# ZHENGXi-git/TC-VIML

Measured on NVIDIA B200. Metric: linearized_factors_per_s, higher is better.
Workload: dtype f64

## Files before the change

### tc-viml_b200/csrc/assemble2.cuh

```cuda
#pragma once

namespace stream {

constexpr int PMAX = 12;
constexpr int FMAXP = 4096;
constexpr int PT = 64;
constexpr int PT_MAX = 512;
constexpr int TASK_T = 180;
constexpr int TASK_F = 24;
constexpr int LTASK = 32;
constexpr int AW = 4;
constexpr int LACC_W = 14;
constexpr int STAGE_D = 1024;
constexpr int LACC_D = TASK_F * LACC_W;
constexpr int WORK_D = STAGE_D + LACC_D + 192;

struct PlanPtrs {
  int4* hdr;
  int4* tasks;
  uint32_t* slots;
  uint32_t* finfo;
  uint32_t* lslots;
  int* any_irregular;
};

__host__ __device__ inline int task_base(int a0_rel, int w, int F) { return a0_rel / 64 + w * (F / TASK_F + PMAX + 4); }

__device__ __forceinline__ int warp_incl_scan(int v, int lane) {
#pragma unroll
  for (int d = 1; d < 32; d <<= 1) {
    const int t = __shfl_up_sync(0xffffffffu, v, d);
    if (lane >= d) v += t;
  }
  return v;
}

__global__ void __launch_bounds__(PT_MAX) plan_kernel(LinearizeArgs A, PlanPtrs PL) {
  extern __shared__ __align__(16) unsigned char plan_raw[];
  __shared__ int gcount[PMAX + 2], grun[PMAX + 2], lcount[PMAX + 1], lrun[PMAX + 1];
  __shared__ int s_bad, s_big, s_ntasks, s_nlslots;
  const int tid = threadIdx.x, lane = tid & 31, warp = tid >> 5, w = blockIdx.x;
  const int P = A.P, F = A.F, NTH = (int)blockDim.x;
  uint32_t* fmask = reinterpret_cast<uint32_t*>(plan_raw);
  uint32_t* fanchor = fmask + F;
  uint32_t* cexcl = fanchor + F;
  uint16_t* ford = reinterpret_cast<uint16_t*>(cexcl + F + 1);
  uint16_t* fid = ford + ((F + 1) & ~1);
  const int a0 = A.pf_window_offset[w], nf = A.pf_window_offset[w + 1] - a0;
  const int b0 = A.NL > 0 ? A.lf_window_offset[w] : 0, nl = A.NL > 0 ? A.lf_window_offset[w + 1] - b0 : 0;
  const int a0r = a0 - (int)A.pf_begin, b0r = b0 - (int)A.lf_begin;
  for (int f = tid; f < F; f += NTH) fmask[f] = 0u, fanchor[f] = 0xffu;
  for (int e = tid; e < F * P; e += NTH) fid[e] = 0xffff;
  if (tid < PMAX + 2) gcount[tid] = 0;
  if (tid < PMAX + 1) lcount[tid] = 0;
  if (tid == 0) s_bad = s_big = (nf > 65534 || nl > 65534 || nf < 0 || nl < 0) ? 1 : 0, s_ntasks = 0, s_nlslots = 0;
  __syncthreads();
  const int nfs = s_big ? 0 : nf;
  for (int k = tid; k < nfs; k += NTH) {
    const uint32_t ix = A.pf_idx[a0 + k];
    const int i = ix & 0xff, j = (ix >> 8) & 0xff, l = ix >> 16;
    if (i >= P || j >= P || l >= F || i == j) {
      s_bad = 1;
      continue;
    }
    const uint32_t old = atomicOr(&fmask[l], 1u << j);
    const uint32_t an = atomicCAS(&fanchor[l], 0xffu, (uint32_t)i);
    if (((old >> j) & 1u) || (an != 0xffu && an != (uint32_t)i)) s_bad = 1;
    fid[l * P + j] = (uint16_t)k;
  }
  __syncthreads();
  if (s_bad) {
    if (tid == 0) {
      PL.hdr[w] = make_int4(0, 0, 1, 0);
      atomicOr(PL.any_irregular, 1);
    }
    return;
  }
  uint32_t* lsl = PL.lslots + 2 * (size_t)b0r;
  if (warp == 0) {
    for (int f0 = 0; f0 < F; f0 += 32) {
      const int f = f0 + lane;
      const int key = f < F ? (fanchor[f] == 0xffu ? P : (int)fanchor[f]) : 64 + lane;
      const unsigned m = __match_any_sync(0xffffffffu, key);
      if (f < F && (m & ((1u << lane) - 1u)) == 0u) gcount[key] += __popc(m);
      __syncwarp();
    }
    {
      const int c = lane <= P ? gcount[lane] : 0;
      const int inc = warp_incl_scan(c, lane);
      if (lane <= P) grun[lane] = inc - c;
    }
    __syncwarp();
    for (int f0 = 0; f0 < F; f0 += 32) {
      const int f = f0 + lane;
      const int key = f < F ? (fanchor[f] == 0xffu ? P : (int)fanchor[f]) : 64 + lane;
      const unsigned m = __match_any_sync(0xffffffffu, key);
      const int rank = __popc(m & ((1u << lane) - 1u));
      if (f < F) ford[grun[key] + rank] = (uint16_t)f;
      __syncwarp();
      if (f < F && rank == 0) grun[key] += __popc(m);
      __syncwarp();
    }
    int carry = 0;
    for (int p0 = 0; p0 < F; p0 += 32) {
      const int p = p0 + lane;
      const int c = p < F ? __popc(fmask[ford[p]]) : 0;
      const int inc = warp_incl_scan(c, lane);
      if (p < F) cexcl[p] = (uint32_t)(carry + inc - c);
      carry += __shfl_sync(0xffffffffu, inc, 31);
    }
    if (lane == 0) cexcl[F] = (uint32_t)carry;
    __syncwarp();
    const int tb = task_base(a0r, w, F);
    int pos = 0, t = 0;
    bool at_group_start = true;
    while (pos < F) {
      const int p = pos + lane;
      const int c = p < F ? (int)(cexcl[p + 1] - cexcl[p]) : 0x10000;
      const int inc = warp_incl_scan(c, lane);
      const unsigned okm = __ballot_sync(0xffffffffu, inc <= TASK_T && p < F && lane < TASK_F);
      int n = okm == 0xffffffffu ? 32 : __ffs(~okm) - 1;
      n = max(n, 1);
      n = min(n, F - pos);
      const int an = p < F ? (fanchor[ford[p]] == 0xffu ? P : (int)fanchor[ford[p]]) : -1;
      const unsigned same = __ballot_sync(0xffffffffu, an == __shfl_sync(0xffffffffu, an, 0));
      const int na = same == 0xffffffffu ? 33 : __ffs(~same) - 1;
      int excl = 0;
      if (na <= n) {
        n = na;
        excl = at_group_start ? 1 : 0;
        at_group_start = true;
      } else {
        at_group_start = false;
      }
      if (lane == 0) PL.tasks[tb + t] = make_int4(2 * (int)cexcl[pos], 0, pos, n | (excl << 16));
      pos += n, ++t;
    }
    if (lane == 0) s_ntasks = t;
  } else if (warp == 1 && nl > 0) {
    bool bad = false;
    for (int k0 = 0; k0 < nl; k0 += 32) {
      const int k = k0 + lane;
      int key = k < nl ? A.lf_frame[b0 + k] : 64 + lane;
      if (k < nl && (key < 0 || key >= P)) bad = true, key = 96 + lane;
      const unsigned m = __match_any_sync(0xffffffffu, key);
      if (k < nl && key < P && (m & ((1u << lane) - 1u)) == 0u) lcount[key] += __popc(m);
      __syncwarp();
    }
    if (__any_sync(0xffffffffu, bad)) {
      if (lane == 0) s_bad = 1;
    } else {
      const int c = lane < P ? ((lcount[lane] + 1) & ~1) : 0;
      const int inc = warp_incl_scan(c, lane);
      if (lane < P) {
        lrun[lane] = inc - c;
        if (lcount[lane] & 1) lsl[inc - 1] = 0xffffu | ((uint32_t)lane << 16);
      }
      if (lane == 31) s_nlslots = inc;
      __syncwarp();
      for (int k0 = 0; k0 < nl; k0 += 32) {
        const int k = k0 + lane;
        const int key = k < nl ? A.lf_frame[b0 + k] : 64 + lane;
        const unsigned m = __match_any_sync(0xffffffffu, key);
        const int rank = __popc(m & ((1u << lane) - 1u));
        if (k < nl) lsl[lrun[key] + rank] = (uint32_t)k | ((uint32_t)key << 16);
        __syncwarp();
        if (k < nl && rank == 0) lrun[key] += __popc(m);
        __syncwarp();
      }
    }
  }
  __syncthreads();
  if (s_bad) {
    if (tid == 0) {
      PL.hdr[w] = make_int4(0, 0, 1, 0);
      atomicOr(PL.any_irregular, 1);
    }
    return;
  }
  const int tb = task_base(a0r, w, F), nt = s_ntasks;
  uint32_t* sl_w = PL.slots + 2 * (size_t)a0r;
  for (int t = warp; t < nt; t += NTH / 32) {
    int4 tk = PL.tasks[tb + t];
    const int p = tk.z + lane;
    const bool on = lane < (tk.w & 0xffff);
    const int l = on ? ford[p] : 0;
    const uint32_t m = on ? fmask[l] : 0u;
    const int an = (on && m) ? (int)fanchor[l] : 0xff;
    if (on) PL.finfo[(size_t)w * F + p] = (uint32_t)l | (m << 16) | ((uint32_t)(an & 15) << 28);
    uint32_t* sl = sl_w + tk.x;
    int off = 0;
    const unsigned lt = (1u << lane) - 1u;
    unsigned im = __reduce_or_sync(0xffffffffu, an < P ? 1u << an : 0u);
    while (im) {
      const int i = __ffs(im) - 1;
      im &= im - 1;
      unsigned jm = __reduce_or_sync(0xffffffffu, an == i ? m : 0u);
      while (jm) {
        const int j = __ffs(jm) - 1;
        jm &= jm - 1;
        const bool mine = an == i && ((m >> j) & 1u);
        const unsigned b = __ballot_sync(0xffffffffu, mine);
        const int n = __popc(b);
        const uint32_t key = ((uint32_t)i << 21) | ((uint32_t)j << 25);
        if (mine) sl[off + __popc(b & lt)] = (uint32_t)fid[l * P + j] | ((uint32_t)lane << 16) | key;
        if ((n & 1) && lane == 0) sl[off + n] = 0xffffu | key;
        off += (n + 1) & ~1;
      }
    }
    if (lane == 0) PL.tasks[tb + t].y = off;
  }
  if (tid == 0) PL.hdr[w] = make_int4(nt, s_nlslots, 0, 0);
}

enum Kind { K_LL = 0, K_HH, K_LH, K_LE, K_HE, K_EE, K_BL, K_BH, K_BE, K_NKIND };

struct Tables {
  uint32_t seg[128];
  uint32_t lo[64];
  uint32_t ee[32];
  uint32_t line[32];
};

constexpr uint32_t tab_entry(int R, int C, int kind, int off, bool neg) {
  const int tile = (R < 8 && C < 8) ? 0 : (R < 8 ? 1 : 2);
  return 0x80000000u | (uint32_t)(tile * 64 + (R & 7) * 8 + (C & 7)) | ((uint32_t)kind << 8) | ((uint32_t)off << 12) |
         (neg ? (1u << 18) : 0u);
}

constexpr int col_type(int c) { return c < 3 ? 0 : (c < 6 ? 1 : (c < 9 ? 2 : (c < 15 ? 3 : 4))); }
// ... 80 lines not shown

__device__ __forceinline__ int swz(int f) { return ((f & 1) << 2) ^ ((f >> 1) & 3); }

struct Dest {
  int src;
  int off;
  int kind;
  unsigned sign;
};
__device__ __forceinline__ Dest decode(uint32_t e) {
  Dest d;
  d.src = (e >> 31) ? (int)(e & 0xff) : -1;
  d.off = (e >> 12) & 63;
  d.kind = (e >> 8) & 15;
  d.sign = ((e >> 18) & 1u) << 31;
  return d;
}
template <int ROUNDS>
__device__ __forceinline__ void scatter(const double* __restrict__ patch, const Dest* tab, double* __restrict__ Hc,
                                        int mybase, bool store_lh = false) {
  double v[ROUNDS];
  double* dst[ROUNDS];
#pragma unroll
  for (int r = 0; r < ROUNDS; ++r) {
    const int base = __shfl_sync(0xffffffffu, mybase, tab[r].kind);
    dst[r] = Hc + base + tab[r].off;
    const double x = patch[tab[r].src >= 0 ? tab[r].src : 0];
    v[r] = __hiloint2double(__double2hiint(x) ^ (int)tab[r].sign, __double2loint(x));
  }
#pragma unroll
  for (int r = 0; r < ROUNDS; ++r) {
    if (tab[r].src >= 0) {
      if (store_lh && tab[r].kind == K_LH) *dst[r] = v[r];
      else atomicAdd(dst[r], v[r]);
    }
  }
}

__device__ __forceinline__ int kind_base(int rs, int cs, bool isb, int lo, int hi, int NB, int boff) {
  const int e = NB - 1;
  const int x = rs == 0 ? lo : (rs == 1 ? hi : e), y = cs == 0 ? lo : (cs == 1 ? hi : e);
  return isb ? boff + 6 * x : blk(x, y, NB) * 36;
}

__device__ __forceinline__ void put_patch(double* __restrict__ patch, int lane, const double (&G)[6]) {
  double2* p2 = reinterpret_cast<double2*>(patch);
  const int o = (lane >> 2) * 4 + (lane & 3);
  p2[o] = make_double2(G[0], G[1]);
  p2[32 + o] = make_double2(G[2], G[3]);
  p2[64 + o] = make_double2(G[4], G[5]);
}

template <bool MODE_A>
__global__ void __maxnreg__(168) assemble_kernel(LinearizeArgs A, PlanPtrs PL, int use_tma) {
  extern __shared__ __align__(16) unsigned char asm_raw[];
  __shared__ int s_next;
  constexpr int NT = AW * 32;
  const int tid = threadIdx.x, lane = tid & 31, warp = tid >> 5, w = blockIdx.x;
  const int P = A.P, F = A.F, D = A.D, NB = P + 1;
  const int nblk = NB * (NB + 1) / 2, boff = nblk * 36;
  const int hc_n = (boff + D + 1) & ~1;
  const int cstride = P * kPoseCache + kExCache;
  double* __restrict__ Hc = reinterpret_cast<double*>(asm_raw);
  double* __restrict__ cache = Hc + hc_n;
  double* __restrict__ work0 = cache + cstride;
  double* __restrict__ stage = work0 + warp * WORK_D;
  double* __restrict__ lacc = stage + STAGE_D;
  double* __restrict__ patch = lacc + LACC_D;

  const int4 hdr = PL.hdr[w];
  const int a0 = A.pf_window_offset[w];
  const int b0 = A.NL > 0 ? A.lf_window_offset[w] : 0;
  double* __restrict__ Hpp = A.out.H_pp + (size_t)w * D * D;
  double* __restrict__ Hlp = A.out.H_lp + (size_t)w * F * D;
  double* __restrict__ Hll = A.out.H_ll + (size_t)w * F;
  double* __restrict__ bp = A.out.b_p + (size_t)w * D;
  double* __restrict__ bl = A.out.b_l + (size_t)w * F;
  const double2* __restrict__ gc = reinterpret_cast<const double2*>(A.cache + (size_t)w * cstride);
  double2 cpre[3];
#pragma unroll
  for (int q = 0; q < 3; ++q) cpre[q] = tid + q * NT < cstride / 2 ? gc[tid + q * NT] : make_double2(0.0, 0.0);
  uint32_t traw[7];
#pragma unroll
  for (int r = 0; r < 3; ++r) traw[r] = g_tables.seg[32 * r + lane];
#pragma unroll
  for (int r = 0; r < 2; ++r) traw[3 + r] = g_tables.lo[32 * r + lane];
  traw[5] = g_tables.ee[lane], traw[6] = g_tables.line[lane];
  if (hdr.z) {
    for (int e = tid; e < D * D; e += NT) Hpp[e] = 0.0;
    for (int e = tid; e < F * D; e += NT) Hlp[e] = 0.0;
    for (int e = tid; e < F; e += NT) Hll[e] = 0.0, bl[e] = 0.0;
    for (int e = tid; e < D; e += NT) bp[e] = 0.0;
    return;
  }
  {
    double2* z = reinterpret_cast<double2*>(Hc);
    for (int e = tid; e < hc_n / 2; e += NT) z[e] = make_double2(0.0, 0.0);
    double2* c2 = reinterpret_cast<double2*>(cache);
#pragma unroll
    for (int q = 0; q < 3; ++q)
      if (tid + q * NT < cstride / 2) c2[tid + q * NT] = cpre[q];
    for (int e = tid + 3 * NT; e < cstride / 2; e += NT) c2[e] = gc[e];
  }
  if (tid == 0) s_next = 0;
  Dest tab_seg[3], tab_lo[2], tab_ee[1], tab_line[1];
#pragma unroll
  for (int r = 0; r < 3; ++r) tab_seg[r] = decode(traw[r]);
#pragma unroll
  for (int r = 0; r < 2; ++r) tab_lo[r] = decode(traw[3 + r]);
  tab_ee[0] = decode(traw[5]);
  tab_line[0] = decode(traw[6]);
  const int kb_rs = lane < K_NKIND ? (0x24904 >> (2 * lane)) & 3 : 0, kb_cs = lane < K_NKIND ? (0xA94 >> (2 * lane)) & 3 : 0;
  const bool kb_isb = lane >= K_BL && lane < K_NKIND;
  __syncthreads();

  const int ntask = hdr.x, nlsl = hdr.y, nltask = (nlsl + LTASK - 1) / LTASK;
  const int tb = task_base(a0 - (int)A.pf_begin, w, F);
  const uint32_t* __restrict__ sl_w = PL.slots + 2 * (size_t)(a0 - (int)A.pf_begin);
  const uint32_t* __restrict__ lsl_w = PL.lslots + 2 * (size_t)(b0 - (int)A.lf_begin);
  const int g = lane >> 2, kk = lane & 3;
  const int gx = g ^ ((kk >> 1) << 2);
  const double* __restrict__ frag0 = stage + (kk >> 1) * 32 + (kk & 1);
  const unsigned full = 0xffffffffu;
  const int upr = 3 * NB;
  const int ru1 = 32 + (lane & 7), rb0 = (lane * 11) >> 5, rb1 = (ru1 * 43) >> 7;
  const int rp0 = lane - 3 * rb0, rp1 = ru1 - 3 * rb1;

  double E[2] = {0.0, 0.0};
  for (;;) {
    int t = 0;
    if (lane == 0) t = atomicAdd(&s_next, 1);
    t = __shfl_sync(full, t, 0);
    if (t >= ntask + nltask) break;
    if (t < ntask) {
      const int4 tk = PL.tasks[tb + t];
      const int n_slots = tk.y, n_feats = tk.w & 0xffff;
      const bool excl = (tk.w >> 16) != 0;
      const uint32_t fi = lane < n_feats ? PL.finfo[(size_t)w * F + tk.z + lane] : 0u;
      {
        double2* z = reinterpret_cast<double2*>(lacc);
        for (int q = lane; q < LACC_D / 2; q += 32) z[q] = make_double2(0.0, 0.0);
      }
      __syncwarp();
      const uint32_t* __restrict__ sl = sl_w + tk.x;
      double G[6] = {0, 0, 0, 0, 0, 0}, R[4] = {0, 0, 0, 0};
// ... 229 lines not shown
      const int br = r / 6, bc = c / 6, rr = r - 6 * br, cc = c - 6 * bc;
      const int lo = min(br, bc), hi = max(br, bc);
      const bool tr = br > bc || (br == bc && rr > cc);
      int a = tr ? cc : rr, b = tr ? rr : cc;
      if (lo != hi && hi < NB - 1 && a < 3 && b < a) { const int t = a; a = b, b = t; }
      Hpp[e] = Hc[blk(lo, hi, NB) * 36 + a * 6 + b];
    }
  } else {
    double2* __restrict__ Hf2 = reinterpret_cast<double2*>(Hf);
    const int Dh = D / 2;
    int br = 0, row0 = 0, rown = NB;
    for (int e = tid; e < nblk * 18; e += NT) {
      const int q = (e * 3641) >> 16, k = e - 18 * q;
      const int rr = (k * 11) >> 5, cp = k - 3 * rr, cc = 2 * cp;
      while (q >= row0 + rown) row0 += rown, --rown, ++br;
      const int bc = br + (q - row0);
      const double* __restrict__ sb = Hc + q * 36;
      if (br != bc) {
        const bool pp = bc < NB - 1;
        auto at = [&](int a, int b) { return sb[(pp && a < 3 && b < a) ? b * 6 + a : a * 6 + b]; };
        Hf2[(6 * br + rr) * Dh + 3 * bc + cp] = make_double2(at(rr, cc), at(rr, cc + 1));
        Hf2[(6 * bc + rr) * Dh + 3 * br + cp] = make_double2(at(cc, rr), at(cc + 1, rr));
      } else {
        Hf2[(6 * br + rr) * Dh + 3 * bc + cp] =
            make_double2(rr <= cc ? sb[rr * 6 + cc] : sb[cc * 6 + rr], rr <= cc + 1 ? sb[rr * 6 + cc + 1] : sb[(cc + 1) * 6 + rr]);
      }
    }
  }
  if (staged) {
    for (int e = tid; e < D; e += NT) Hf[D * D + e] = Hc[boff + e];
  } else {
    for (int e = tid; e < D; e += NT) bp[e] = Hc[boff + e];
  }
  if (use_tma) {
    asm volatile("fence.proxy.async.shared::cta;" ::: "memory");
    __syncthreads();
    if (tid == 0) {
      const uint32_t s0 = (uint32_t)__cvta_generic_to_shared(Hf);
      asm volatile("cp.async.bulk.global.shared::cta.bulk_group [%0], [%1], %2;" ::"l"(Hpp), "r"(s0), "r"((uint32_t)(D * D * 8))
                   : "memory");
      asm volatile("cp.async.bulk.global.shared::cta.bulk_group [%0], [%1], %2;" ::"l"(bp), "r"(s0 + (uint32_t)(D * D * 8)),
                   "r"((uint32_t)(D * 8))
                   : "memory");
      asm volatile("cp.async.bulk.commit_group;" ::: "memory");
      asm volatile("cp.async.bulk.wait_group.read 0;" ::: "memory");
    }
  } else if (staged) {
    __syncthreads();
    for (int e = tid; e < D * D; e += NT) Hpp[e] = Hf[e];
    for (int e = tid; e < D; e += NT) bp[e] = Hf[D * D + e];
  }
}

template <bool MODE_A>
__global__ void __launch_bounds__(128) irregular_kernel(LinearizeArgs A, PlanPtrs PL) {
  if (!*PL.any_irregular) return;
  const int cstride = A.P * kPoseCache + kExCache;
  for (int w = blockIdx.x; w < A.W; w += gridDim.x) {
    if (!PL.hdr[w].z) continue;
    const double* cw = A.cache + (size_t)w * cstride;
    const int a0 = A.pf_window_offset[w], a1 = A.pf_window_offset[w + 1];
    for (int64_t k = a0 + threadIdx.x; k < a1; k += blockDim.x) {
      const uint32_t pk = A.pf_idx[k];
      const int i = pk & 0xff, j = (pk >> 8) & 0xff, f = pk >> 16;
      if (i >= A.P || j >= A.P || f >= A.F) continue;
      const double4 ob = reinterpret_cast<const double4*>(A.pf_obs)[k];
      const double piz = A.pf_pts_i_z ? A.pf_pts_i_z[k] : 1.0;
      PointJac J;
      eval_point(A, cw, i, j, A.inv_depth[(size_t)w * A.F + f], ob.x, ob.y, piz, ob.z, ob.w, J);
      if (MODE_A) {
        if (A.out.pf_residual) reinterpret_cast<double2*>(A.out.pf_residual)[k] = make_double2(J.r[0], J.r[1]);
        if (A.out.pf_jac_pose_i) store_jac7(A.out.pf_jac_pose_i + 14 * k, J.a);
        if (A.out.pf_jac_pose_j) store_jac7(A.out.pf_jac_pose_j + 14 * k, J.b);
        if (A.out.pf_jac_ex) store_jac7(A.out.pf_jac_ex + 14 * k, J.c);
        if (A.out.pf_jac_feat) reinterpret_cast<double2*>(A.out.pf_jac_feat)[k] = make_double2(J.d[0], J.d[1]);
      }
      point_atomics(A, w, i, j, f, J, true, false);
    }
    if (A.NL > 0) {
      const int b0 = A.lf_window_offset[w], b1 = A.lf_window_offset[w + 1];
      for (int64_t k = b0 + threadIdx.x; k < b1; k += blockDim.x) {
        const int frame = A.lf_frame[k];
        if (frame < 0 || frame >= A.P) continue;
        double g9[9];
#pragma unroll
        for (int c = 0; c < 9; ++c) g9[c] = A.lf_geom[(size_t)c * A.NL_stride + k];
        LineJac J;
        eval_line(A, cw, frame, g9, J);
        if (MODE_A) {
          if (A.out.lf_residual) reinterpret_cast<double2*>(A.out.lf_residual)[k] = make_double2(J.r[0], J.r[1]);
          if (A.out.lf_jac_pose) store_jac7(A.out.lf_jac_pose + 14 * k, J.a);
        }
        line_atomics(A, w, frame, J);
      }
    }
  }
}

}
```

### tc-viml_b200/csrc/common.cuh

```cuda
#pragma once
#include <cuda_runtime.h>

#include <cstdint>
#include <cstdio>
#include <string>
#include <utility>
#include <vector>

#include "viml.h"

#define VIML_TRY_CUDA(ctx, expr)                                                              \
  do {                                                                                        \
    cudaError_t e__ = (expr);                                                                 \
    if (e__ != cudaSuccess) {                                                                 \
      (ctx)->err = std::string(#expr) + ": " + cudaGetErrorString(e__);                      \
      return VIML_ERR_CUDA;                                                                   \
    }                                                                                         \
  } while (0)

struct DeviceArena {
  char* base = nullptr;
  size_t cap = 0, used = 0;
  cudaError_t reserve(size_t bytes) {
    used = 0;
// ... 10 lines not shown
  T* take(size_t count) {
    const size_t bytes = (count * sizeof(T) + 255) & ~size_t(255);
    T* p = (T*)(base + used);
    used += bytes;
    return p;
  }
  static size_t padded(size_t bytes) { return (bytes + 255) & ~size_t(255); }
  void release() {
    if (base) cudaFree(base);
    base = nullptr;
    cap = used = 0;
  }
};

struct viml_ctx {
  int device = 0;
  int sm_count = 148;
  cudaStream_t stream = nullptr;
  cudaStream_t copy_stream = nullptr;
  cudaStream_t copy_stream2 = nullptr;
  cudaEvent_t ev_a = nullptr, ev_b = nullptr;
  cudaStream_t aux_stream = nullptr;
  cudaEvent_t ev_fork = nullptr, ev_join = nullptr;
  viml_config cfg{};
  std::string err;
  int64_t launches = 0;
  double cos_th = 0.0;
  int nan_angle_passes = 0;
  double* d_map = nullptr;
  int64_t n_map = 0;
  bool map_set = false;
  double* d_map_sorted = nullptr;
  int32_t* d_map_orig = nullptr;
  double* d_tile_sphere = nullptr;
  double* d_group_sphere = nullptr;
  int64_t n_tiles = 0;
  uint32_t* d_fov_slots = nullptr;
  int32_t* d_fov_slot_count = nullptr;
  int64_t fov_words = 0;
  unsigned long long* d_assoc_stats = nullptr;
  DeviceArena in_arena, out_arena, scratch, scratch2, scratch3, gn_in, gn_out, s_full;
  bool schur_splitk = false;
  char *h_stage_in = nullptr, *h_stage_out = nullptr;
  size_t h_stage_in_cap = 0, h_stage_out_cap = 0;
  void* nccl_lib = nullptr;
  bool brute_cull = false;
  bool force_generic = false;
  bool prof = false;
  std::vector<std::pair<cudaEvent_t, cudaEvent_t>> prof_events[VIML_NUM_KERNELS];
};

enum KernelId {
  K_PREP = 0, K_POINTS, K_LINES, K_ASSEMBLE, K_SCHUR, K_CAMPOSE, K_CULL, K_SCAN, K_FILL, K_PROJECT, K_MATCH,
  K_MARG, K_MICRO, K_PLAN, K_IRREGULAR, K_GN, K_COUNT
};
static_assert(K_COUNT <= VIML_NUM_KERNELS, "raise VIML_NUM_KERNELS");

struct LaunchScope {
  viml_ctx* ctx;
  cudaEvent_t stop = nullptr;
  cudaStream_t on;
  LaunchScope(viml_ctx* c, int id, cudaStream_t st = nullptr) : ctx(c), on(st ? st : c->stream) {
    ctx->launches++;
    if (ctx->prof) {
      cudaEvent_t a, b;
      cudaEventCreate(&a);
      cudaEventCreate(&b);
      cudaEventRecord(a, on);
      ctx->prof_events[id].emplace_back(a, b);
      stop = b;
    }
  }
  ~LaunchScope() {
    if (stop) cudaEventRecord(stop, on);
  }
};

constexpr int kMapTile = 64;
constexpr int kPoseCache = 42;
constexpr int kExCache = 24;
constexpr int PC_P = 0, PC_R = 3, PC_RINV = 12, PC_M = 21, PC_RL = 30, PC_TL = 39;
constexpr int EC_TIC = 0, EC_RIC = 3, EC_RICINV = 12, EC_RTT = 21;

struct LinearizeArgs {
  int W, P, F, D;
  int64_t NP, NL;
  int64_t pf_begin, lf_begin;
  int64_t NL_stride;
  const double* poses;
  const double* ex_pose;
  const double* inv_depth;
  const int32_t* pf_window_offset;
  const uint32_t* pf_idx;
  const double* pf_obs;
  const double* pf_pts_i_z;
  const int32_t* lf_window_offset;
  const int32_t* lf_frame;
  const double* lf_geom;
  double* cache;
  viml_linearize_out out;
  double sqrt_info, cauchy_a, inv_cauchy_a2, fx, fy, cx, cy;
  uint32_t flags;
};

struct DenseArgs {
  int X;
  int64_t ND;
// ... 102 lines not shown
```

### tc-viml_b200/csrc/linearize_kernels.cu

```cuda
#include <cstdlib>
#include <vector>

#include "common.cuh"

namespace {

__device__ __forceinline__ void quat_to_rot(double w, double x, double y, double z, double* R) {
  const double tx = 2.0 * x, ty = 2.0 * y, tz = 2.0 * z;
  const double twx = tx * w, twy = ty * w, twz = tz * w;
  const double txx = tx * x, txy = ty * x, txz = tz * x;
  const double tyy = ty * y, tyz = tz * y, tzz = tz * z;
  R[0] = 1.0 - (tyy + tzz);
  R[1] = txy - twz;
  R[2] = txz + twy;
  R[3] = txy + twz;
  R[4] = 1.0 - (txx + tzz);
  R[5] = tyz - twx;
  R[6] = txz - twy;
  R[7] = tyz + twx;
  R[8] = 1.0 - (txx + tyy);
}

__device__ __forceinline__ void mul_AtBt(const double* A, const double* B, double* C) {
#pragma unroll
// ... 410 lines not shown

template <bool MODE_A, bool MODE_B>
__global__ void __launch_bounds__(128) lines_kernel(LinearizeArgs A) {
  __shared__ double2 stage[MODE_A ? 4 * 7 * 32 : 1];
  const int64_t k_raw = A.lf_begin + blockIdx.x * (int64_t)blockDim.x + threadIdx.x;
  const int64_t k_end = A.lf_begin + A.NL;
  const int lane = threadIdx.x & 31;
  const int64_t k_warp = k_raw - lane;
  if (k_warp >= k_end) return;
  const int nvalid = (int)min((int64_t)32, k_end - k_warp);
  const int64_t k = min(k_raw, k_end - 1);
  const bool live = k_raw < k_end;
  const int w = find_window_warp(A.lf_window_offset, A.W, k, k_warp);
  const int frame = A.lf_frame[k];
  double g9[9];
#pragma unroll
  for (int c = 0; c < 9; ++c) g9[c] = A.lf_geom[(size_t)c * A.NL_stride + k];
  const double* cw = A.cache + (size_t)w * (A.P * kPoseCache + kExCache);
  LineJac J;
  eval_line(A, cw, frame, g9, J);
  if (MODE_A) {
    if (live && A.out.lf_residual) reinterpret_cast<double2*>(A.out.lf_residual)[k] = make_double2(J.r[0], J.r[1]);
    if (A.out.lf_jac_pose)
      store_jac7_coalesced(stage + (threadIdx.x >> 5) * 7 * 32, A.out.lf_jac_pose + 14 * k_warp, J.a, lane, nvalid);
  }
  if (MODE_B && live) line_atomics(A, w, frame, J);
}

__global__ void __launch_bounds__(256) pack_upper_kernel(int D, const double* __restrict__ S, double* __restrict__ Sp) {
  const double* __restrict__ s = S + (size_t)blockIdx.x * D * D;
  double* __restrict__ o = Sp + (size_t)blockIdx.x * ((size_t)D * (D + 1) / 2);
  for (int e = blockIdx.y * blockDim.x + threadIdx.x; e < D * D; e += gridDim.y * blockDim.x) {
    const int r = e / D, c = e - r * D;
    if (c >= r) o[(size_t)r * D - ((size_t)r * (r - 1)) / 2 + c - r] = s[e];
  }
}

#include "assemble2.cuh"
#include "gn_kernels.cuh"

}

int viml_launch_linearize(viml_ctx* ctx, const LinearizeArgs& a) {
  cudaStream_t st = ctx->stream;
  const bool modeA = (a.flags & VIML_OUT_RESIDUAL_JACOBIAN) != 0;
  const bool modeB = (a.flags & (VIML_OUT_HB | VIML_OUT_SCHUR)) != 0;
  const size_t plan_smem = (size_t)a.F * 8 + ((size_t)a.F + 1) * 4 + (((size_t)a.F + 1) & ~(size_t)1) * 2 + (size_t)a.F * a.P * 2 + 16;
  const bool fast = modeB && a.P <= stream::PMAX && a.F <= stream::FMAXP && plan_smem <= 200 * 1024 && !ctx->force_generic;
  stream::PlanPtrs PL{};
  if (fast) {
    const size_t n_tasks = (size_t)a.NP / 64 + (size_t)a.W * (a.F / stream::TASK_F + stream::PMAX + 4) + 2;
    auto pad = [](size_t b) { return DeviceArena::padded(b); };
    VIML_TRY_CUDA(ctx, ctx->scratch3.reserve(pad((size_t)a.W * 16) + pad(n_tasks * 16) + pad((size_t)a.NP * 8 + 8) +
                                             pad((size_t)a.W * a.F * 4 + 4) + pad((size_t)a.NL * 8 + 8) + pad(4)));
    PL.hdr = ctx->scratch3.take<int4>((size_t)a.W);
    PL.tasks = ctx->scratch3.take<int4>(n_tasks);
    PL.slots = ctx->scratch3.take<uint32_t>((size_t)a.NP * 2 + 2);
    PL.finfo = ctx->scratch3.take<uint32_t>((size_t)a.W * a.F + 1);
    PL.lslots = ctx->scratch3.take<uint32_t>((size_t)a.NL * 2 + 2);
    PL.any_irregular = ctx->scratch3.take<int>(1);
    VIML_TRY_CUDA(ctx, cudaEventRecord(ctx->ev_fork, st));
    VIML_TRY_CUDA(ctx, cudaStreamWaitEvent(ctx->aux_stream, ctx->ev_fork, 0));
    VIML_TRY_CUDA(ctx, cudaMemsetAsync(PL.any_irregular, 0, 4, ctx->aux_stream));
    VIML_TRY_CUDA(ctx, cudaFuncSetAttribute(stream::plan_kernel, cudaFuncAttributeMaxDynamicSharedMemorySize, (int)plan_smem));
    {
      LaunchScope ls(ctx, K_PLAN, ctx->aux_stream);
      stream::plan_kernel<<<a.W, a.F > 512 ? stream::PT_MAX : stream::PT, plan_smem, ctx->aux_stream>>>(a, PL);
    }
    VIML_TRY_CUDA(ctx, cudaEventRecord(ctx->ev_join, ctx->aux_stream));
  }
  {
    const int64_t total = (int64_t)a.W * (a.P + 1);
    LaunchScope ls(ctx, K_PREP);
    prep_windows_kernel<<<(unsigned)((total + 127) / 128), 128, 0, st>>>(a);
  }
  if (fast) {
    VIML_TRY_CUDA(ctx, cudaStreamWaitEvent(st, ctx->ev_join, 0));
    const int NB = a.P + 1, nblk = NB * (NB + 1) / 2;
    const size_t smem = ((size_t)((nblk * 36 + a.D + 1) & ~1) + (size_t)a.P * kPoseCache + kExCache + (size_t)stream::AW * stream::WORK_D) * 8;
    const int use_tma = ((((uintptr_t)a.out.H_pp) | ((uintptr_t)a.out.b_p)) & 15) == 0 ? 1 : 0;
    VIML_TRY_CUDA(ctx, cudaFuncSetAttribute(stream::assemble_kernel<true>, cudaFuncAttributeMaxDynamicSharedMemorySize, (int)smem));
    VIML_TRY_CUDA(ctx, cudaFuncSetAttribute(stream::assemble_kernel<false>, cudaFuncAttributeMaxDynamicSharedMemorySize, (int)smem));
    {
      LaunchScope ls(ctx, K_ASSEMBLE);
      if (modeA) stream::assemble_kernel<true><<<a.W, stream::AW * 32, smem, st>>>(a, PL, use_tma);
      else stream::assemble_kernel<false><<<a.W, stream::AW * 32, smem, st>>>(a, PL, use_tma);
    }
    {
      const int grid = a.W < 4 * ctx->sm_count ? a.W : 4 * ctx->sm_count;
      LaunchScope ls(ctx, K_IRREGULAR);
      if (modeA) stream::irregular_kernel<true><<<grid, 128, 0, st>>>(a, PL);
      else stream::irregular_kernel<false><<<grid, 128, 0, st>>>(a, PL);
    }
  } else {
    if (modeB) {
      const size_t W = a.W, D = a.D, F = a.F;
      VIML_TRY_CUDA(ctx, cudaMemsetAsync(a.out.H_pp, 0, W * D * D * sizeof(double), st));
      VIML_TRY_CUDA(ctx, cudaMemsetAsync(a.out.H_lp, 0, W * F * D * sizeof(double), st));
      VIML_TRY_CUDA(ctx, cudaMemsetAsync(a.out.H_ll, 0, W * F * sizeof(double), st));
      VIML_TRY_CUDA(ctx, cudaMemsetAsync(a.out.b_p, 0, W * D * sizeof(double), st));
      VIML_TRY_CUDA(ctx, cudaMemsetAsync(a.out.b_l, 0, W * F * sizeof(double), st));
    }
    if (a.NP > 0) {
      const unsigned grid = (unsigned)((a.NP + 127) / 128);
      LaunchScope ls(ctx, K_POINTS);
      if (modeA && modeB) points_kernel<true, true><<<grid, 128, 0, st>>>(a);
      else if (modeA) points_kernel<true, false><<<grid, 128, 0, st>>>(a);
      else if (modeB) points_kernel<false, true><<<grid, 128, 0, st>>>(a);
    }
    if (a.NL > 0) {
      const unsigned grid = (unsigned)((a.NL + 127) / 128);
      LaunchScope ls(ctx, K_LINES);
      if (modeA && modeB) lines_kernel<true, true><<<grid, 128, 0, st>>>(a);
      else if (modeA) lines_kernel<true, false><<<grid, 128, 0, st>>>(a);
      else if (modeB) lines_kernel<false, true><<<grid, 128, 0, st>>>(a);
    }
  }
  if (a.flags & VIML_OUT_SCHUR) {
    const double eps = 1e-8;
    double* S = a.out.S;
    if (a.flags & VIML_S_PACKED) {
      VIML_TRY_CUDA(ctx, ctx->s_full.reserve(DeviceArena::padded((size_t)a.W * a.D * a.D * 8)));
      S = ctx->s_full.take<double>((size_t)a.W * a.D * a.D);
    }
    viml_launch_schur(ctx, a.W, a.F, a.D, a.out.H_pp, a.out.H_lp, a.out.H_ll, a.out.b_p, a.out.b_l, S, a.out.g, eps);
    if (a.flags & VIML_S_PACKED) {
      LaunchScope ls(ctx, K_SCHUR);
      const unsigned slices = (unsigned)std::min<int64_t>(((int64_t)a.D * a.D + 256 * 32 - 1) / (256 * 32), 1024);
      pack_upper_kernel<<<dim3((unsigned)a.W, slices), 256, 0, st>>>(a.D, S, a.out.S);
    }
  }
  VIML_TRY_CUDA(ctx, cudaGetLastError());
  return VIML_OK;
}

int viml_launch_expand_obs(viml_ctx* ctx, const LinearizeArgs& a, const void* feat_obs, const void* pf_obs_j, bool f32) {
  if (a.NP == 0) return VIML_OK;
  LaunchScope ls(ctx, K_PREP);
  if (f32) expand_obs_kernel<float2><<<a.W, 128, 0, ctx->stream>>>(a, (const float2*)feat_obs, (const float2*)pf_obs_j);
  else expand_obs_kernel<double2><<<a.W, 128, 0, ctx->stream>>>(a, (const double2*)feat_obs, (const double2*)pf_obs_j);
  VIML_TRY_CUDA(ctx, cudaGetLastError());
  return VIML_OK;
}

int viml_launch_expand_lines(viml_ctx* ctx, const LinearizeArgs& a, const int32_t* lf_map_index, const float* lf_seg2d) {
  if (a.NL == 0) return VIML_OK;
// ... 76 lines not shown
```

### tc-viml_b200/csrc/viml_api.cu

```cuda
#include <dlfcn.h>

#include <cmath>
#include <cstdlib>
#include <algorithm>
#include <cstring>
#include <ctime>
#include <numeric>
#include <vector>

#include "common.cuh"

namespace {

thread_local std::string g_create_error;

double cos_threshold(double angle_th) {
  if (!(std::acos(1.0) <= angle_th)) return INFINITY;
  if (std::acos(0.0) <= angle_th) return 0.0;
  uint64_t lo, hi;
  double dlo = 0.0, dhi = 1.0;
  std::memcpy(&lo, &dlo, 8);
  std::memcpy(&hi, &dhi, 8);
  while (hi - lo > 1) {
    const uint64_t mid = lo + (hi - lo) / 2;
// ... 116 lines not shown
  VIML_TRY_CUDA(ctx, cudaSetDevice(ctx->device));
  VIML_TRY_CUDA(ctx, cudaMalloc(p, bytes));
  return VIML_OK;
}
int viml_device_free(viml_ctx* ctx, void* p) {
  if (!ctx) return VIML_ERR_INVALID;
  VIML_TRY_CUDA(ctx, cudaSetDevice(ctx->device));
  VIML_TRY_CUDA(ctx, cudaFree(p));
  return VIML_OK;
}
int viml_memcpy_h2d(viml_ctx* ctx, void* dst, const void* src, size_t bytes) {
  if (!ctx) return VIML_ERR_INVALID;
  VIML_TRY_CUDA(ctx, cudaMemcpyAsync(dst, src, bytes, cudaMemcpyHostToDevice, ctx->stream));
  return VIML_OK;
}
int viml_memcpy_d2h(viml_ctx* ctx, void* dst, const void* src, size_t bytes) {
  if (!ctx) return VIML_ERR_INVALID;
  VIML_TRY_CUDA(ctx, cudaMemcpyAsync(dst, src, bytes, cudaMemcpyDeviceToHost, ctx->stream));
  return VIML_OK;
}

int64_t viml_kernel_launches(const viml_ctx* ctx) { return ctx ? ctx->launches : 0; }


int viml_profile_begin(viml_ctx* ctx) {
  if (!ctx) return VIML_ERR_INVALID;
  VIML_TRY_CUDA(ctx, cudaSetDevice(ctx->device));
  drop_prof_events(ctx);
  ctx->prof = true;
  return VIML_OK;
}

int viml_profile_end(viml_ctx* ctx, double* ms, int64_t* n) {
  if (!ctx) return VIML_ERR_INVALID;
  ctx->prof = false;
  VIML_TRY_CUDA(ctx, cudaStreamSynchronize(ctx->stream));
  for (int k = 0; k < VIML_NUM_KERNELS; ++k) {
    double tot = 0.0;
    for (auto& pr : ctx->prof_events[k]) {
      float t = 0.f;
      if (cudaEventElapsedTime(&t, pr.first, pr.second) == cudaSuccess) tot += t;
    }
    if (ms) ms[k] = tot;
    if (n) n[k] = (int64_t)ctx->prof_events[k].size();
  }
  drop_prof_events(ctx);
  return VIML_OK;
}

const char* viml_kernel_name(int id) {
  static const char* names[VIML_NUM_KERNELS] = {"prep_windows", "linearize_points", "linearize_lines", "assemble_hb",
                                                "schur_landmarks", "assoc_cam_pose", "assoc_cull", "assoc_scan",
                                                "assoc_fill_list", "assoc_project", "assoc_match", "marginalize_dense",
                                                "microbench", "plan_windows", "assemble_irregular", "gn_step"};
  return (id >= 0 && id < VIML_NUM_KERNELS) ? names[id] : "";
}

int viml_set_map(viml_ctx* ctx, const double* lines, int64_t n) {
  if (!ctx || n < 0 || (n > 0 && !lines)) return VIML_ERR_INVALID;
  VIML_TRY_CUDA(ctx, cudaSetDevice(ctx->device));
  VIML_TRY_CUDA(ctx, cudaStreamSynchronize(ctx->stream));
  auto drop = [&](auto*& ptr) {
    if (ptr) cudaFree(ptr);
    ptr = nullptr;
  };
  drop(ctx->d_map), drop(ctx->d_map_sorted), drop(ctx->d_map_orig), drop(ctx->d_tile_sphere), drop(ctx->d_group_sphere);
  drop(ctx->d_fov_slots), drop(ctx->d_fov_slot_count);
  ctx->fov_words = 0;
  ctx->n_map = 0, ctx->n_tiles = 0;
  ctx->map_set = true;
  if (n == 0) return VIML_OK;
  std::vector<double> soa((size_t)6 * n);
  for (int64_t j = 0; j < n; ++j)
    for (int c = 0; c < 6; ++c) soa[(size_t)c * n + j] = lines[6 * j + c];
  VIML_TRY_CUDA(ctx, cudaMalloc((void**)&ctx->d_map, soa.size() * sizeof(double)));
  VIML_TRY_CUDA(ctx, cudaMemcpy(ctx->d_map, soa.data(), soa.size() * sizeof(double), cudaMemcpyHostToDevice));
  double lo[3] = {INFINITY, INFINITY, INFINITY}, hi[3] = {-INFINITY, -INFINITY, -INFINITY};
  for (int64_t j = 0; j < n; ++j)
    for (int c = 0; c < 3; ++c) {
      const double m = 0.5 * (lines[6 * j + c] + lines[6 * j + 3 + c]);
      if (std::isfinite(m)) lo[c] = std::min(lo[c], m), hi[c] = std::max(hi[c], m);
    }
  auto spread = [](uint64_t v) {
    v &= 0x1fffff;
    v = (v | v << 32) & 0x1f00000000ffffull;
    v = (v | v << 16) & 0x1f0000ff0000ffull;
    v = (v | v << 8) & 0x100f00f00f00f00full;
    v = (v | v << 4) & 0x10c30c30c30c30c3ull;
    v = (v | v << 2) & 0x1249249249249249ull;
    return v;
  };
  double span = 0.0;
  for (int c = 0; c < 3; ++c)
    if (hi[c] > lo[c]) span = std::max(span, hi[c] - lo[c]);
  if (!(span > 0.0)) span = 1.0;
  std::vector<uint64_t> key(n);
  for (int64_t j = 0; j < n; ++j) {
    uint64_t k = 0;
    for (int c = 0; c < 3; ++c) {
      const double m = 0.5 * (lines[6 * j + c] + lines[6 * j + 3 + c]);
      double t = std::isfinite(m) ? (m - lo[c]) / span : 0.0;
      t = std::min(1.0, std::max(0.0, t));
      k |= spread((uint64_t)(t * 2097151.0)) << c;
    }
    key[j] = k;
  }
  std::vector<int32_t> order(n);
// ... 735 lines not shown
```

Baseline: 5.516 billion.

## Fold irregular-window fallback into assemble kernel and drop separate launch

Windows flagged as irregular by the planner are now handled inside the assemble kernel itself, right after their outputs are zeroed, instead of by a separate irregular_kernel launch that checked a global flag. The any_irregular flag, its memset and its atomics go away, along with the fid initialisation loop in the planner. This removes one kernel launch, one memset and a flag read per call in the common all-regular case. In exchange, irregular windows now run with the assemble kernel's small block and stage a PointJac through shared memory. Dropping the fid reset assumes nothing reads stale fid entries.

```diff
diff --git a/profiles/compare_dumps.py b/profiles/compare_dumps.py
--- /dev/null
+++ b/profiles/compare_dumps.py
@@ -0,0 +1,31 @@
+import os
+import sys
+
+import numpy as np
+
+sys.path.insert(0, os.path.dirname(os.path.dirname(os.path.abspath(__file__))))
+import __graft_entry__ as ge
+
+BIT_EXACT = ("H_lp", "H_ll", "b_l")
+ROUNDING = {"H_pp": 1e-12, "b_p": 1e-12}
+
+
+def main(a, b):
+    parity = ge.load_package().parity
+    ok = True
+    for k in BIT_EXACT + tuple(ROUNDING):
+        x, y = np.load(os.path.join(a, k + ".npy")), np.load(os.path.join(b, k + ".npy"))
+        if k in BIT_EXACT:
+            same = x.shape == y.shape and np.array_equal(x.view(np.uint64), y.view(np.uint64))
+            print(f"{k:5s} {x.shape} bit-identical: {same}")
+            ok &= same
+        else:
+            e = parity.unit_err(k, x, y)
+            print(f"{k:5s} {x.shape} max unit error {e:.3e} (bar {ROUNDING[k]:.0e})")
+            ok &= e < ROUNDING[k]
+    print("PASS" if ok else "FAIL")
+    return 0 if ok else 1
+
+
+if __name__ == "__main__":
+    sys.exit(main(sys.argv[1], sys.argv[2]))
diff --git a/tc-viml_b200/csrc/assemble2.cuh b/tc-viml_b200/csrc/assemble2.cuh
--- a/tc-viml_b200/csrc/assemble2.cuh
+++ b/tc-viml_b200/csrc/assemble2.cuh
@@ -21,7 +21,6 @@
   uint32_t* slots;
   uint32_t* finfo;
   uint32_t* lslots;
-  int* any_irregular;
 };
 
 __host__ __device__ inline int task_base(int a0_rel, int w, int F) { return a0_rel / 64 + w * (F / TASK_F + PMAX + 4); }
@@ -50,7 +49,6 @@
   const int b0 = A.NL > 0 ? A.lf_window_offset[w] : 0, nl = A.NL > 0 ? A.lf_window_offset[w + 1] - b0 : 0;
   const int a0r = a0 - (int)A.pf_begin, b0r = b0 - (int)A.lf_begin;
   for (int f = tid; f < F; f += NTH) fmask[f] = 0u, fanchor[f] = 0xffu;
-  for (int e = tid; e < F * P; e += NTH) fid[e] = 0xffff;
   if (tid < PMAX + 2) gcount[tid] = 0;
   if (tid < PMAX + 1) lcount[tid] = 0;
   if (tid == 0) s_bad = s_big = (nf > 65534 || nl > 65534 || nf < 0 || nl < 0) ? 1 : 0, s_ntasks = 0, s_nlslots = 0;
@@ -70,10 +68,7 @@
   }
   __syncthreads();
   if (s_bad) {
-    if (tid == 0) {
-      PL.hdr[w] = make_int4(0, 0, 1, 0);
-      atomicOr(PL.any_irregular, 1);
-    }
+    if (tid == 0) PL.hdr[w] = make_int4(0, 0, 1, 0);
     return;
   }
   uint32_t* lsl = PL.lslots + 2 * (size_t)b0r;
@@ -172,10 +167,7 @@
   }
   __syncthreads();
   if (s_bad) {
-    if (tid == 0) {
-      PL.hdr[w] = make_int4(0, 0, 1, 0);
-      atomicOr(PL.any_irregular, 1);
-    }
+    if (tid == 0) PL.hdr[w] = make_int4(0, 0, 1, 0);
     return;
   }
   const int tb = task_base(a0r, w, F), nt = s_ntasks;
@@ -362,6 +354,48 @@
 }
 
 template <bool MODE_A>
+__device__ void assemble_irregular(const LinearizeArgs& A, int w, int tid, int NT, PointJac* Js) {
+  const double* cw = A.cache + (size_t)w * (A.P * kPoseCache + kExCache);
+  const int a0 = A.pf_window_offset[w], a1 = A.pf_window_offset[w + 1];
+  for (int64_t k = a0 + tid; k < a1; k += NT) {
+    const uint32_t pk = A.pf_idx[k];
+    const int i = pk & 0xff, j = (pk >> 8) & 0xff, f = pk >> 16;
+    if (i >= A.P || j >= A.P || f >= A.F) continue;
+    const double4 ob = reinterpret_cast<const double4*>(A.pf_obs)[k];
+    const double piz = A.pf_pts_i_z ? A.pf_pts_i_z[k] : 1.0;
+    PointJac J;
+    eval_point(A, cw, i, j, A.inv_depth[(size_t)w * A.F + f], ob.x, ob.y, piz, ob.z, ob.w, J);
+    if (MODE_A) {
+      if (A.out.pf_residual) reinterpret_cast<double2*>(A.out.pf_residual)[k] = make_double2(J.r[0], J.r[1]);
+      if (A.out.pf_jac_pose_i) store_jac7(A.out.pf_jac_pose_i + 14 * k, J.a);
+      if (A.out.pf_jac_pose_j) store_jac7(A.out.pf_jac_pose_j + 14 * k, J.b);
+      if (A.out.pf_jac_ex) store_jac7(A.out.pf_jac_ex + 14 * k, J.c);
+      if (A.out.pf_jac_feat) reinterpret_cast<double2*>(A.out.pf_jac_feat)[k] = make_double2(J.d[0], J.d[1]);
+    }
+    *Js = J;
+    __threadfence_block();
+    point_atomics(A, w, i, j, f, *Js, true, false);
+  }
+  if (A.NL > 0) {
+    const int b0 = A.lf_window_offset[w], b1 = A.lf_window_offset[w + 1];
+    for (int64_t k = b0 + tid; k < b1; k += NT) {
+      const int frame = A.lf_frame[k];
+      if (frame < 0 || frame >= A.P) continue;
+      double g9[9];
+#pragma unroll
+      for (int c = 0; c < 9; ++c) g9[c] = A.lf_geom[(size_t)c * A.NL_stride + k];
+      LineJac J;
+      eval_line(A, cw, frame, g9, J);
+      if (MODE_A) {
+        if (A.out.lf_residual) reinterpret_cast<double2*>(A.out.lf_residual)[k] = make_double2(J.r[0], J.r[1]);
+        if (A.out.lf_jac_pose) store_jac7(A.out.lf_jac_pose + 14 * k, J.a);
+      }
+      line_atomics(A, w, frame, J);
+    }
+  }
+}
+
+template <bool MODE_A>
 __global__ void __maxnreg__(168) assemble_kernel(LinearizeArgs A, PlanPtrs PL, int use_tma) {
   extern __shared__ __align__(16) unsigned char asm_raw[];
   __shared__ int s_next;
@@ -401,6 +435,8 @@
     for (int e = tid; e < F * D; e += NT) Hlp[e] = 0.0;
     for (int e = tid; e < F; e += NT) Hll[e] = 0.0, bl[e] = 0.0;
     for (int e = tid; e < D; e += NT) bp[e] = 0.0;
+    __syncthreads();
+    assemble_irregular<MODE_A>(A, w, tid, NT, reinterpret_cast<PointJac*>(stage) + lane);
     return;
   }
   {
@@ -736,49 +772,4 @@
   }
 }
 
-template <bool MODE_A>
-__global__ void __launch_bounds__(128) irregular_kernel(LinearizeArgs A, PlanPtrs PL) {
-  if (!*PL.any_irregular) return;
-  const int cstride = A.P * kPoseCache + kExCache;
-  for (int w = blockIdx.x; w < A.W; w += gridDim.x) {
-    if (!PL.hdr[w].z) continue;
-    const double* cw = A.cache + (size_t)w * cstride;
-    const int a0 = A.pf_window_offset[w], a1 = A.pf_window_offset[w + 1];
-    for (int64_t k = a0 + threadIdx.x; k < a1; k += blockDim.x) {
-      const uint32_t pk = A.pf_idx[k];
-      const int i = pk & 0xff, j = (pk >> 8) & 0xff, f = pk >> 16;
-      if (i >= A.P || j >= A.P || f >= A.F) continue;
-      const double4 ob = reinterpret_cast<const double4*>(A.pf_obs)[k];
-      const double piz = A.pf_pts_i_z ? A.pf_pts_i_z[k] : 1.0;
-      PointJac J;
-      eval_point(A, cw, i, j, A.inv_depth[(size_t)w * A.F + f], ob.x, ob.y, piz, ob.z, ob.w, J);
-      if (MODE_A) {
-        if (A.out.pf_residual) reinterpret_cast<double2*>(A.out.pf_residual)[k] = make_double2(J.r[0], J.r[1]);
-        if (A.out.pf_jac_pose_i) store_jac7(A.out.pf_jac_pose_i + 14 * k, J.a);
-        if (A.out.pf_jac_pose_j) store_jac7(A.out.pf_jac_pose_j + 14 * k, J.b);
-        if (A.out.pf_jac_ex) store_jac7(A.out.pf_jac_ex + 14 * k, J.c);
-        if (A.out.pf_jac_feat) reinterpret_cast<double2*>(A.out.pf_jac_feat)[k] = make_double2(J.d[0], J.d[1]);
-      }
-      point_atomics(A, w, i, j, f, J, true, false);
-    }
-    if (A.NL > 0) {
-      const int b0 = A.lf_window_offset[w], b1 = A.lf_window_offset[w + 1];
-      for (int64_t k = b0 + threadIdx.x; k < b1; k += blockDim.x) {
-        const int frame = A.lf_frame[k];
-        if (frame < 0 || frame >= A.P) continue;
-        double g9[9];
-#pragma unroll
-        for (int c = 0; c < 9; ++c) g9[c] = A.lf_geom[(size_t)c * A.NL_stride + k];
-        LineJac J;
-        eval_line(A, cw, frame, g9, J);
-        if (MODE_A) {
-          if (A.out.lf_residual) reinterpret_cast<double2*>(A.out.lf_residual)[k] = make_double2(J.r[0], J.r[1]);
-          if (A.out.lf_jac_pose) store_jac7(A.out.lf_jac_pose + 14 * k, J.a);
-        }
-        line_atomics(A, w, frame, J);
-      }
-    }
-  }
-}
-
-}
+}
diff --git a/tc-viml_b200/csrc/common.cuh b/tc-viml_b200/csrc/common.cuh
--- a/tc-viml_b200/csrc/common.cuh
+++ b/tc-viml_b200/csrc/common.cuh
@@ -86,7 +86,7 @@
 
 enum KernelId {
   K_PREP = 0, K_POINTS, K_LINES, K_ASSEMBLE, K_SCHUR, K_CAMPOSE, K_CULL, K_SCAN, K_FILL, K_PROJECT, K_MATCH,
-  K_MARG, K_MICRO, K_PLAN, K_IRREGULAR, K_GN, K_COUNT
+  K_MARG, K_MICRO, K_PLAN, K_GN, K_COUNT
 };
 static_assert(K_COUNT <= VIML_NUM_KERNELS, "raise VIML_NUM_KERNELS");
 
diff --git a/tc-viml_b200/csrc/linearize_kernels.cu b/tc-viml_b200/csrc/linearize_kernels.cu
--- a/tc-viml_b200/csrc/linearize_kernels.cu
+++ b/tc-viml_b200/csrc/linearize_kernels.cu
@@ -486,16 +486,14 @@
     const size_t n_tasks = (size_t)a.NP / 64 + (size_t)a.W * (a.F / stream::TASK_F + stream::PMAX + 4) + 2;
     auto pad = [](size_t b) { return DeviceArena::padded(b); };
     VIML_TRY_CUDA(ctx, ctx->scratch3.reserve(pad((size_t)a.W * 16) + pad(n_tasks * 16) + pad((size_t)a.NP * 8 + 8) +
-                                             pad((size_t)a.W * a.F * 4 + 4) + pad((size_t)a.NL * 8 + 8) + pad(4)));
+                                             pad((size_t)a.W * a.F * 4 + 4) + pad((size_t)a.NL * 8 + 8)));
     PL.hdr = ctx->scratch3.take<int4>((size_t)a.W);
     PL.tasks = ctx->scratch3.take<int4>(n_tasks);
     PL.slots = ctx->scratch3.take<uint32_t>((size_t)a.NP * 2 + 2);
     PL.finfo = ctx->scratch3.take<uint32_t>((size_t)a.W * a.F + 1);
     PL.lslots = ctx->scratch3.take<uint32_t>((size_t)a.NL * 2 + 2);
-    PL.any_irregular = ctx->scratch3.take<int>(1);
     VIML_TRY_CUDA(ctx, cudaEventRecord(ctx->ev_fork, st));
     VIML_TRY_CUDA(ctx, cudaStreamWaitEvent(ctx->aux_stream, ctx->ev_fork, 0));
-    VIML_TRY_CUDA(ctx, cudaMemsetAsync(PL.any_irregular, 0, 4, ctx->aux_stream));
     VIML_TRY_CUDA(ctx, cudaFuncSetAttribute(stream::plan_kernel, cudaFuncAttributeMaxDynamicSharedMemorySize, (int)plan_smem));
     {
       LaunchScope ls(ctx, K_PLAN, ctx->aux_stream);
@@ -520,12 +518,6 @@
       if (modeA) stream::assemble_kernel<true><<<a.W, stream::AW * 32, smem, st>>>(a, PL, use_tma);
       else stream::assemble_kernel<false><<<a.W, stream::AW * 32, smem, st>>>(a, PL, use_tma);
     }
-    {
-      const int grid = a.W < 4 * ctx->sm_count ? a.W : 4 * ctx->sm_count;
-      LaunchScope ls(ctx, K_IRREGULAR);
-      if (modeA) stream::irregular_kernel<true><<<grid, 128, 0, st>>>(a, PL);
-      else stream::irregular_kernel<false><<<grid, 128, 0, st>>>(a, PL);
-    }
   } else {
     if (modeB) {
       const size_t W = a.W, D = a.D, F = a.F;
diff --git a/tc-viml_b200/csrc/viml_api.cu b/tc-viml_b200/csrc/viml_api.cu
--- a/tc-viml_b200/csrc/viml_api.cu
+++ b/tc-viml_b200/csrc/viml_api.cu
@@ -192,7 +192,7 @@
   static const char* names[VIML_NUM_KERNELS] = {"prep_windows", "linearize_points", "linearize_lines", "assemble_hb",
                                                 "schur_landmarks", "assoc_cam_pose", "assoc_cull", "assoc_scan",
                                                 "assoc_fill_list", "assoc_project", "assoc_match", "marginalize_dense",
-                                                "microbench", "plan_windows", "assemble_irregular", "gn_step"};
+                                                "microbench", "plan_windows", "gn_step"};
   return (id >= 0 && id < VIML_NUM_KERNELS) ? names[id] : "";
 }
 
```

Result: faster. 5.601 billion, median of 6 (+1.5%).
